# ZhengyiLuo/UHC

Hardware: NVIDIA H100
Metric: env_steps_per_s (higher is better)
Workload: dtype f32

## Files before the change

### include/uhc_b200.h

```cpp
#ifndef UHC_B200_H
#define UHC_B200_H
#ifdef __cplusplus
extern "C" {
#endif

#define UHC_NB 24
#define UHC_NQ 76
#define UHC_NV 75
#define UHC_NU 69
#define UHC_OBS_DIM 657
#define UHC_ACT_DIM 105
#define UHC_MAX_ACT_DIM 315
#define UHC_OBS_DIM_V1 784
#define UHC_EX_SIZE 576
#define UHC_BODYF 20

typedef struct UhcEngine UhcEngine;

typedef struct {
    int nvert, nnbr;
    const double *body_f;
    const double *dof_f;
    const double *hull;
    const int *hull_adr, *hull_num, *nbr, *nbradr;
// ... 38 lines not shown
int uhc_load_motions_time(const UhcEngine *e, float *out2);

int uhc_set_clip_models(UhcEngine *e, int nclips, const int *clip_model);

int uhc_set_neutral_pose(UhcEngine *e, const double *qpos76, const double *qvel75);

int uhc_set_clip_weights(UhcEngine *e, int nclips, const float *weights_host);
int uhc_get_clip_cdf(UhcEngine *e, float *out_host);

int uhc_env_reset(UhcEngine *e, int n, const int *env_ids_host, const int *clip_host, const int *start_host, const int *len_host,
                  const float *qpos_dev, const float *qvel_dev, float *obs_dev, void *stream);

int uhc_env_step(UhcEngine *e, const float *actions_dev, float *obs_dev, float *reward_dev, float *cinfo_dev, int *fail_dev,
                 int *end_dev, float *percent_dev, float *torque_dev, void *stream);

int uhc_env_step_host(UhcEngine *e, const float *actions_host, float *obs_host, float *reward_host, float *cinfo_host,
                      int *fail_host, int *end_host, float *percent_host);

int uhc_env_get_state(UhcEngine *e, int env, double *qpos76, double *qvel75, double *xpos72, double *bquat96, int *istate8);
int uhc_env_set_state(UhcEngine *e, int env, const double *qpos76, const double *qvel75);
int uhc_env_get_state_batch(UhcEngine *e, int n, const int *env_ids_host, double *out_host, int *istate_host);
int uhc_env_set_state_batch(UhcEngine *e, int n, const int *env_ids_host, const double *qpos_host, const double *qvel_host);
int uhc_engine_counters(UhcEngine *e, int *out4);
const int *uhc_episode_log_dev(const UhcEngine *e);
int uhc_num_envs(const UhcEngine *e);
int uhc_engine_obs_dim(const UhcEngine *e);
int uhc_engine_act_dim(const UhcEngine *e);
int uhc_kernel_launches(const UhcEngine *e);

#ifdef __cplusplus
}
#endif
#endif
```

### uhc_b200/build.py

```python
import os
import subprocess
import tempfile

HERE = os.path.dirname(os.path.abspath(__file__))
SO = os.path.join(HERE, "libuhc_b200.so")
SRCS = ["step_kernel.cu", "nn_kernels.cu", "mlp_wgmma.cu", "rollout.cu", "ppo_update.cu"]
NO_FMA_SRCS = ["motion_lib.cu", "eval.cu", "curriculum.cu", "track.cu", "export.cu"]
DEPS = ["sim_core.h", "env_step.h", "motion_core.h", "eval_core.h", "eval_glue.h", "group_core.h", "curriculum_core.h", "track_core.h", "track_obs.h", "track_glue.h", "smpl_export_core.h", "../../include/uhc_b200.h", "../../include/uhc_nn.h", "../../include/uhc_rollout.h", "../../include/uhc_ppo.h", "../../include/uhc_eval.h", "../../include/uhc_track.h", "../../include/uhc_export.h"]
NVCC_FLAGS = ["-gencode", "arch=compute_90a,code=sm_90a", "-O3", "-lineinfo", "-std=c++17", "--use_fast_math=false",
              "-Xcompiler", "-fPIC", "-shared", "-Xptxas", "-v", "--expt-relaxed-constexpr"]


def build(force=False, verbose=False):
    csrc = os.path.join(HERE, "csrc")
    srcs = [os.path.join(csrc, s) for s in SRCS]
    nofma = [os.path.join(csrc, s) for s in NO_FMA_SRCS]
    deps = srcs + nofma + [os.path.join(csrc, d) for d in DEPS] + [os.path.abspath(__file__)]
    if not force and os.path.exists(SO) and os.path.getmtime(SO) >= max(os.path.getmtime(d) for d in deps if os.path.exists(d)):
        return SO
    flags = [f for f in NVCC_FLAGS if f != "--use_fast_math=false"] + os.environ.get("UHC_NVCC_EXTRA", "").split()
    with tempfile.TemporaryDirectory() as tmp:
        objs = []
        for s in nofma:
            o = os.path.join(tmp, os.path.basename(s) + ".o")
            cmd = ["nvcc"] + [f for f in flags if f != "-shared"] + ["-fmad=false", "-c", "-o", o, s]
            r = subprocess.run(cmd, capture_output=True, text=True)
            if verbose or r.returncode:
                print(r.stdout[-6000:], r.stderr[-12000:])
            if r.returncode:
                raise RuntimeError("nvcc failed")
            objs.append(o)
        cmd = ["nvcc"] + flags + ["-o", SO] + srcs + objs + ["-ldl"]
        r = subprocess.run(cmd, capture_output=True, text=True)
    if verbose or r.returncode:
        print(r.stdout[-6000:], r.stderr[-12000:])
    if r.returncode:
        raise RuntimeError("nvcc failed")
    return SO


if __name__ == "__main__":
    build(force=True, verbose=True)
```

### uhc_b200/csrc/env_step.h

```cpp
#pragma once
#include "sim_core.h"
#include "curriculum_core.h"

namespace uhc {

struct CurView {
    const float *pct;
    const int *start;
    const int *meta;
    int max_freq, fit_clip;
    float prec_freq;
};

template <class Real>
struct EngineView {
    Model<Real> model;
    EnvCfg<Real> cfg;
    int num_envs;
    Real *state;
    int *istate;
    const Real *expert;
    const int *clip_adr;
    const Real *clip_shape;
    const int *clip_model;
// ... 100 lines not shown
UHC_DEV unsigned smem_u32(const void *p) { return (unsigned)__cvta_generic_to_shared(p); }
template <class Real>
UHC_DEV void state_mbar_init(Work<Real> &w) {
    if ((threadIdx.x & 31) == 0) {
        asm volatile("mbarrier.init.shared::cta.b64 [%0], 1;" :: "r"(smem_u32(&w.mbar)));
        asm volatile("fence.mbarrier_init.release.cluster;" ::: "memory");
    }
    __syncwarp();
}
template <class Real>
UHC_DEV void copy16(Real *dst, const Real *src, int n) {
    const int nv = n * (int)sizeof(Real) / 16;
    for (int i = threadIdx.x & 31; i < nv; i += 32) reinterpret_cast<uint4 *>(dst)[i] = reinterpret_cast<const uint4 *>(src)[i];
}
#endif
template <class Real>
UHC_DEV void load_state(const EngineView<Real> &ev, int env, Work<Real> &w, int parity) {
    const Real *st = ev.state + (size_t)env * ST_SIZE;
#ifndef UHC_EMU
    constexpr unsigned BYTES = ST_BLOCK * sizeof(Real);
    static_assert(BYTES % 16 == 0 && (ST_SIZE * sizeof(Real)) % 16 == 0, "bulk copies need 16-byte granularity");
    const unsigned mb = smem_u32(&w.mbar);
    if ((threadIdx.x & 31) == 0) {
        asm volatile("mbarrier.arrive.expect_tx.shared::cta.b64 _, [%0], %1;" :: "r"(mb), "r"(BYTES) : "memory");
        asm volatile("cp.async.bulk.shared::cluster.global.mbarrier::complete_tx::bytes [%0], [%1], %2, [%3];"
                     :: "r"(smem_u32(w.q)), "l"(st), "r"(BYTES), "r"(mb) : "memory");
    }
    unsigned done = 0;
    while (!done) {
        asm volatile("{ .reg .pred p; mbarrier.try_wait.parity.shared::cta.b64 p, [%1], %2; selp.u32 %0, 1, 0, p; }" : "=r"(done) : "r"(mb), "r"(parity) : "memory");
    }
    __syncwarp();
#else
    (void)parity;
    { Real *head = reinterpret_cast<Real *>(&w); for (int i = 0; i < ST_BLOCK; i++) head[i] = st[i]; }
#endif
}
template <class Real>
UHC_DEV void store_state(const EngineView<Real> &ev, int env, Work<Real> &w) {
    Real *st = ev.state + (size_t)env * ST_SIZE;
#ifndef UHC_EMU
    constexpr unsigned BYTES = ST_BLOCK * sizeof(Real);
    __syncwarp();
    copy16(st + ST_XPOS, &w.xpos[0][0], 72); copy16(st + ST_XIPOS, &w.xipos[0][0], 72); copy16(st + ST_XQUAT, &w.xquat[0][0], 96);
    if ((threadIdx.x & 31) == 0) {
        asm volatile("fence.proxy.async.shared::cta;" ::: "memory");
// ... 34 lines not shown
    }
    LANES_BEGIN
    if (lane == 0) { w.mdl = model_for_clip(ev, clip); w.cfg = ev.cfg; w.con_overflow = 0; }
    LANES_END
    const Model<Real> &mdl = w.mdl;
    TOPO_DECL(mdl);
    const int iters = substep_dynamics<Real, ObsT>(mdl, w.cfg, w, tp, (const Real *)nullptr, 0, false, (ObsT *)nullptr);
    world_quat(mdl, w.q, w);
    int *is = ev.istate + (size_t)env * SI_SIZE;
    Real *st = ev.state + (size_t)env * ST_SIZE;
    LANES_BEGIN
    for (int i = lane; i < 96; i += 32) { const Real v = (i & 3) == 0 ? Real(1) : Real(0); st[ST_BQUAT + i] = v; st[ST_PBQUAT + i] = v; }
    if (lane == 0) { is[SI_CUR_T] = 0; is[SI_CLIP] = clip; is[SI_START] = start; is[SI_LEN] = len; is[SI_NEWTON] = iters; is[SI_NCON] = w.ncon; }
    LANES_END
    if (obs) write_obs(ev, w, clip, start, len, 1, obs);
    LANES_BEGIN
    for (int i = lane; i < NV; i += 32) w.aw[i] = 0;
    LANES_END
    store_state(ev, env, w);
}

template <class Real, class ObsT, bool CUR = false>
UHC_DEV int env_step_warp(const EngineView<Real> &ev, int env, Work<Real> &w, const ObsT *action, ObsT *obs, ObsT *reward,
                          ObsT *cinfo_out, int *fail_out, int *end_out, ObsT *percent_out, ObsT *torque_out) {
    int *is = ev.istate + (size_t)env * SI_SIZE;
    Real *st = ev.state + (size_t)env * ST_SIZE;
    const int clip = is[SI_CLIP], start = is[SI_START], len = is[SI_LEN];
    int cur_t = is[SI_CUR_T];
    load_state(ev, env, w, 0);
    const bool explicit_rf = ev.cfg.rfc_mode == 1;
    LANES_BEGIN
    for (int i = lane; i < NU; i += 32) w.act[i] = (Real)action[i];
    if (lane < 6) w.act[NU + lane] = ev.cfg.rfc_mode == 0 ? (Real)action[NU + lane] : Real(0);
    if (lane < 2 * NSUB) w.act[NU + 6 + lane] = ev.cfg.meta_pd ? (Real)action[NU + ev.cfg.vf_dim + lane] : Real(0);
    LANES_END
    if (explicit_rf) restore_stale_pose(w, st + ST_XPOS, st + ST_XQUAT);
    const Real *target = expert_frame(ev, clip, start, len, cur_t + 1) + EX_QPOS + 7;
    int iters = 0, maxcon = 0;
    LANES_BEGIN
    if (lane == 0) { w.mdl = model_for_clip(ev, clip); w.cfg = ev.cfg; w.con_overflow = 0; }
    LANES_END
    const Model<Real> &mdl = w.mdl;
    TOPO_DECL(mdl);
#pragma unroll 1
    for (int it = 0; it < NSUB; ++it) {
        UHC_CTA_SYNC(true);
        iters += substep_dynamics<Real, ObsT>(mdl, w.cfg, w, tp, target, it, true, torque_out, true, action);
        if (w.ncon > maxcon) maxcon = w.ncon;
        if (it == NSUB - 1) world_quat(mdl, w.q, w);
        integrate(mdl, w);
    }
    cur_t += 1;
    Real *bq = st + ST_BQUAT, *pbq = st + ST_PBQUAT;
    LANES_BEGIN
    for (int i = lane; i < 96; i += 32) pbq[i] = bq[i];
    LANES_END
    body_quat(w, bq);
    Real bd, rew, ci[5];
    const Real *exf = expert_frame(ev, clip, start, len, cur_t);
    diff_and_reward(mdl, w.cfg, w, exf, bq, pbq, &bd, &rew, ci, action);
    int fail;
    if (ev.cfg.term_body == 0) fail = bd > ev.cfg.body_diff_thresh;
    else {
        const Real *f0 = ev.expert + (size_t)(UHC_LDG(ev.clip_adr + clip) + start) * EX_SIZE;
        const int off = ev.cfg.term_body == 1 ? EX_QPOS + 2 : EX_WBPOS + 3 * ev.cfg.head_body + 2;
        LVAR(Real, neg);
        LANES_BEGIN
        Real mx = Real(-1e30);
        for (int i = lane; i < len; i += 32) { const Real z = -(Real)UHC_LDG(f0 + (size_t)i * EX_SIZE + off); mx = z > mx ? z : mx; }
        LV(neg) = mx;
        LANES_END
        const Real lb = -WMAX(neg);
        fail = (ev.cfg.term_body == 1 ? w.q[2] : w.xpos[ev.cfg.head_body][2]) < lb - Real(0.1);
// ... 25 lines not shown
            const float pctf = (float)((Real)cur_t / (Real)(len - 1));
            ev.ep_log[2 * env] = (fail || end) ? clip : -1;
#ifndef UHC_EMU
            ev.ep_log[2 * env + 1] = __float_as_int(pctf);
#else
            union { float f; int i; } cv; cv.f = pctf; ev.ep_log[2 * env + 1] = cv.i;
#endif
            if constexpr (CUR) ev.ep_start_log[env] = start;
        }
    }
    if (cinfo_out && lane < 5) cinfo_out[lane] = (ObsT)ci[lane];
    LANES_END
    store_state(ev, env, w);
    if (ev.cfg.auto_reset && (fail || end)) {
        int nclip, nstart, nlen;
        const int episode = is[SI_EPISODE] + 1;
        if constexpr (CUR) sample_clip_cur(ev, env, episode, &nclip, &nstart, &nlen);
        else sample_clip(ev, env, episode, &nclip, &nstart, &nlen);
        env_reset_warp<Real, ObsT>(ev, env, w, nclip, nstart, nlen, (const Real *)nullptr, (const Real *)nullptr, obs);
        LANES_BEGIN
        if (lane == 0) is[SI_EPISODE] = episode;
        LANES_END
    }
    return fail || end;
}

}
```

### uhc_b200/csrc/sim_core.h

```cpp
#pragma once
#include <math.h>
#include <stdint.h>

#ifndef UHC_EMU
#include <cuda_runtime.h>
#define UHC_DEV __device__ __forceinline__
#define UHC_DEVNI __device__ __noinline__
#define LANES_BEGIN { const int lane = (int)(threadIdx.x & 31);
#define LANES_END } __syncwarp();
#define LANES_END_R }
#define LVAR(T, n) T n
#define LV(n) n
#define LVARA(T, n, K) T n[K]
#define LVA(n) n
#define LV_ARR(n, c) n[c]
#define LV_ALL(n) n
#define UHC_LDG(p) __ldg(p)
__device__ __forceinline__ float uhc_lds(const float *p) { float v; asm("ld.shared.f32 %0, [%1];" : "=f"(v) : "r"((unsigned)__cvta_generic_to_shared(p))); return v; }
__device__ __forceinline__ double uhc_lds(const double *p) { double v; asm("ld.shared.f64 %0, [%1];" : "=d"(v) : "r"((unsigned)__cvta_generic_to_shared(p))); return v; }
__device__ __forceinline__ int uhc_lds(const int *p) { int v; asm("ld.shared.s32 %0, [%1];" : "=r"(v) : "r"((unsigned)__cvta_generic_to_shared(p))); return v; }
#define UHC_LDT(p) uhc_lds(p)
#else
#define UHC_DEV static inline
#define UHC_DEVNI static
// ... 1088 lines not shown
    const Real dt = m.dt;
    LANES_BEGIN
    for (int i = lane; i < NV; i += 32) { const Real vn = w.v[i] + dt * w.a[i]; w.v[i] = vn; w.aw[i] = w.a[i]; if (i >= 6) w.q[i + 1] += dt * vn; }
    LANES_END
    LANES_BEGIN
    if (lane < 3) w.q[lane] += dt * w.v[lane];
    if (lane == 3) {
        const Real wx = w.v[3], wy = w.v[4], wz = w.v[5], n = sqrt(wx * wx + wy * wy + wz * wz), ang = n * dt;
        Real dq[4] = {1, 0, 0, 0}, qn[4], qo[4] = {w.q[3], w.q[4], w.q[5], w.q[6]};
        if (ang > Real(1e-30)) { Real sn, cs; sincos_(Real(0.5) * ang, &sn, &cs); const Real s = sn / n; dq[0] = cs; dq[1] = wx * s; dq[2] = wy * s; dq[3] = wz * s; }
        qmul(qo, dq, qn);
        const Real nn = rsqrt_(qn[0] * qn[0] + qn[1] * qn[1] + qn[2] * qn[2] + qn[3] * qn[3]);
        for (int i = 0; i < 4; i++) w.q[3 + i] = qn[i] * nn;
    }
    LANES_END
}

enum { PH_PD = 0, PH_SMOOTH = 1, PH_NEWTON = 2 };
#if !defined(UHC_EMU) && !defined(UHC_NO_CTA_SYNC)
#define UHC_CTA_SYNC(on) do { if (on) asm volatile("bar.sync %0, %1;" :: "r"(w.sync_id), "r"(w.sync_threads) : "memory"); } while (0)
#else
#define UHC_CTA_SYNC(on) do { (void)(on); } while (0)
#endif
template <class Real, class OutT, class TPT>
UHC_DEVNI int substep_dynamics(const Model<Real> &m, const EnvCfg<Real> &cfg, Work<Real> &w, const TPT &tp, const Real *target, int it,
                             bool with_pd, OutT *torque_out, bool cta_sync = false, const OutT *act_global = nullptr) {
    int phase = with_pd ? PH_PD : PH_SMOOTH, iters = 0;
    bool done = false;
    Real scale = 0, gn2 = 0;
    for (;;) {
        Real *rhs = w.p;
        Real arm_scale = 0;
        if (phase == PH_PD) {
            pd_setup(m, cfg, w, target, it);
            Real sp, sd; pd_gains(cfg, w, it, &sp, &sd);
            arm_scale = sd * m.dt;
        } else if (phase == PH_SMOOTH) {
            Real fapp[6] = {0, 0, 0, 0, 0, 0};
            const bool explicit_rf = with_pd && cfg.rfc_mode == 1 && act_global != nullptr;
            if (explicit_rf) rfc_explicit(m, cfg, w, tp, act_global, w.as_);
            else if (with_pd && cfg.rfc_mode == 0) rfc_implicit(cfg, w, fapp);
            kin_rne_forward(m, w, tp);
            project_force(m, w, w.Fb, w.C, Real(1), (const Real *)nullptr);
            collide(m, w, tp);
            LANES_BEGIN
            for (int i = lane; i < NV; i += 32) {
                Real f = -w.C[i];
                if (explicit_rf) f += w.as_[i];
                else if (i < 6) { const Real fa = i == 0 ? fapp[0] : i == 1 ? fapp[1] : i == 2 ? fapp[2] : i == 3 ? fapp[3] : i == 4 ? fapp[4] : fapp[5]; f += fa; }
                if (i >= 6 && with_pd) f += w.tau[i - 6];
                w.fs[i] = f; w.as_[i] = f;
            }
            LANES_END
            rhs = w.as_;
            limit_setup(m, w);
        } else {
            if (done || iters >= cfg.newton_max_iter || !(gn2 > cfg.newton_tol * cfg.newton_tol * scale * scale)) break;
            ++iters;
        }
        if (!(phase == PH_SMOOTH && (w.ncon > 0 || w.nlim > 0))) aba_solve(m, w, arm_scale, phase == PH_NEWTON, rhs);
        if (phase == PH_PD) { pd_finish(m, cfg, w, it, torque_out); phase = PH_SMOOTH; UHC_CTA_SYNC(cta_sync); }
        else if (phase == PH_SMOOTH) {
            UHC_CTA_SYNC(cta_sync);
            if (w.ncon == 0 && w.nlim == 0) {
                LANES_BEGIN
                for (int i = lane; i < NV; i += 32) w.a[i] = w.as_[i];
                LANES_END
                done = true;
            } else {
                constraint_setup(m, w);
                scale = newton_init(m, w, tp, &gn2);
            }
            phase = PH_NEWTON;
        } else if (newton_advance(m, w, tp, &gn2)) done = true;
    }
    return iters;
}

template <class Real>
UHC_DEVNI void body_quat(const Work<Real> &w, Real *out) {
    LANES_BEGIN
    const int b = lane;
    if (b == 0) for (int i = 0; i < 4; i++) out[i] = w.q[3 + i];
    else if (b < NB) euler_zyx_quat(w.q[7 + 3 * (b - 1)], w.q[8 + 3 * (b - 1)], w.q[9 + 3 * (b - 1)], out + 4 * b);
    LANES_END
}
template <class Real>
UHC_DEVNI void world_quat(const Model<Real> &m, const Real *qfk, Work<Real> &w) {
    LANES_BEGIN
    const int b = lane;
    if (b < NB) {
        int chain[MAXLEVEL + 1], n = 0;
        for (int a = b; a > 0; a = UHC_LDG(m.parent + a)) chain[n++] = a;
        Real q[4] = {qfk[3], qfk[4], qfk[5], qfk[6]};
        const Real nn = rsqrt_(q[0] * q[0] + q[1] * q[1] + q[2] * q[2] + q[3] * q[3]);
// ... 209 lines not shown
```

### uhc_b200/csrc/step_kernel.cu

```cuda
#include <cuda_runtime.h>
#include <stdio.h>
#include <stdlib.h>
#include <string.h>
#include <string>
#include <vector>
#include "../../include/uhc_b200.h"
#include "../../include/uhc_rollout.h"
#include "env_step.h"
#include "motion_core.h"
#include "eval_glue.h"
#include "curriculum_core.h"
#include "track_obs.h"
#include "track_glue.h"

using namespace uhc;

static thread_local std::string g_err;
#define CK(x) do { cudaError_t e_ = (x); if (e_ != cudaSuccess) { g_err = std::string(#x) + ": " + cudaGetErrorString(e_); return -1; } } while (0)

template <class Real, int EPB>
__device__ __forceinline__ void stage_tables(EngineView<Real> &ev, unsigned char *smem) {
    Real *s_dof = reinterpret_cast<Real *>(smem + EPB * sizeof(Work<Real>));
    Real *s_lim = s_dof + NV * 4;
    int *s_lvl = reinterpret_cast<int *>(s_lim + NV * 4);
    for (int i = threadIdx.x; i < NV * 4; i += blockDim.x) { s_dof[i] = ev.model.dof_f[i]; s_lim[i] = ev.model.dof_lim[i]; }
    for (int i = threadIdx.x; i < (MAXLEVEL + 1) * LVL_G; i += blockDim.x) s_lvl[i] = ev.model.lvl_pack[i];
    LaneTopo *s_topo = reinterpret_cast<LaneTopo *>(s_lvl + (MAXLEVEL + 1) * LVL_G);
    if (threadIdx.x < 32) s_topo[threadIdx.x] = lane_topo(ev.model, (int)threadIdx.x);
    __syncthreads();
    ev.model.dof_f = s_dof; ev.model.dof_lim = s_lim; ev.model.lvl_pack = s_lvl; ev.model.topo_s = s_topo;
}

constexpr int SYNC_GROUP = 8;
#ifdef UHC_MAXNREG
#define UHC_STEP_BOUNDS(EPB, Real) __maxnreg__(UHC_MAXNREG)
#else
#define UHC_STEP_BOUNDS(EPB, Real) __launch_bounds__(32 * EPB, 1)
#endif
template <class Real, int EPB, bool CUR = false>
__global__ void UHC_STEP_BOUNDS(EPB, Real)
k_env_step(EngineView<Real> ev, const float *__restrict__ act, float *__restrict__ obs, float *__restrict__ rew, float *__restrict__ cinfo,
           int *__restrict__ fail, int *__restrict__ end, float *__restrict__ pct, float *__restrict__ torque, const int *__restrict__ order) {
    extern __shared__ __align__(16) unsigned char smem[];
    constexpr int NGRP = (EPB + SYNC_GROUP - 1) / SYNC_GROUP;
    __shared__ int s_nvalid[NGRP];
    const int warp = threadIdx.x >> 5, slot = blockIdx.x * EPB + warp, grp = warp / SYNC_GROUP;
    if (threadIdx.x < NGRP) s_nvalid[threadIdx.x] = 0;
    stage_tables<Real, EPB>(ev, smem);
    const int env = slot < ev.num_envs ? (order ? order[slot] : slot) : -1;
    const bool valid = env >= 0 && env_record_valid(ev, env);
    if (valid && (threadIdx.x & 31) == 0) atomicAdd(&s_nvalid[grp], 1);
    __syncthreads();
    if (!valid) {
        if (env >= 0) env_step_invalid<Real, float>(ev, obs ? obs + (size_t)env * ev.cfg.obs_dim : nullptr, rew ? rew + env : nullptr, cinfo ? cinfo + (size_t)env * 5 : nullptr,
                                                    fail ? fail + env : nullptr, end ? end + env : nullptr, pct ? pct + env : nullptr);
        return;
    }
    Work<Real> &w = reinterpret_cast<Work<Real> *>(smem)[warp];
    if ((threadIdx.x & 31) == 0) { w.sync_threads = 32 * s_nvalid[grp]; w.sync_id = 1 + grp; }
    state_mbar_init(w);
    env_step_warp<Real, float, CUR>(ev, env, w, act + (size_t)env * ev.cfg.act_dim, obs ? obs + (size_t)env * ev.cfg.obs_dim : nullptr, rew ? rew + env : nullptr,
                               cinfo ? cinfo + (size_t)env * 5 : nullptr, fail ? fail + env : nullptr, end ? end + env : nullptr,
                               pct ? pct + env : nullptr, torque ? torque + (size_t)env * NSUB * NU : nullptr);
}

__global__ void __launch_bounds__(1024) k_order_envs(const int *__restrict__ istate, int E, int *__restrict__ order) {
    __shared__ int hist[64], base[64];
    if (threadIdx.x < 64) hist[threadIdx.x] = 0;
    __syncthreads();
    for (int i = threadIdx.x; i < E; i += blockDim.x) { int k = istate[(size_t)i * SI_SIZE + SI_NEWTON]; k = k < 0 ? 0 : (k > 63 ? 63 : k); atomicAdd(&hist[k], 1); }
    __syncthreads();
    if (threadIdx.x == 0) { int run = 0; for (int k = 0; k < 64; k++) { base[k] = run; run += hist[k]; } }
    __syncthreads();
    for (int i = threadIdx.x; i < E; i += blockDim.x) { int k = istate[(size_t)i * SI_SIZE + SI_NEWTON]; k = k < 0 ? 0 : (k > 63 ? 63 : k); order[atomicAdd(&base[k], 1)] = i; }
}

template <class Real, int EPB>
__global__ void __launch_bounds__(32 * EPB)
k_env_reset(EngineView<Real> ev, int n, const int *__restrict__ ids, const int *__restrict__ clip, const int *__restrict__ start,
            const int *__restrict__ len, const float *__restrict__ qpos, const float *__restrict__ qvel, float *__restrict__ obs) {
    extern __shared__ __align__(16) unsigned char smem[];
    const int warp = threadIdx.x >> 5, i = blockIdx.x * EPB + warp;
    stage_tables<Real, EPB>(ev, smem);
    if (i >= n) return;
    Work<Real> &w = reinterpret_cast<Work<Real> *>(smem)[warp];
    const int env = ids[i];
// ... 59 lines not shown
template <class Real>
__global__ void k_gather_state(const Real *__restrict__ state, const int *__restrict__ istate, const int *__restrict__ ids, int n, double *__restrict__ out, int *__restrict__ iout) {
    const int i = blockIdx.x; if (i >= n) return;
    const int env = ids[i];
    const Real *st = state + (size_t)env * ST_SIZE;
    double *o = out + (size_t)i * 319;
    for (int k = threadIdx.x; k < NQ; k += blockDim.x) o[k] = (double)st[ST_Q + k];
    for (int k = threadIdx.x; k < NV; k += blockDim.x) o[76 + k] = (double)st[ST_V + k];
    for (int k = threadIdx.x; k < 72; k += blockDim.x) o[151 + k] = (double)st[ST_XPOS + k];
    for (int k = threadIdx.x; k < 96; k += blockDim.x) o[223 + k] = (double)st[ST_BQUAT + k];
    if (threadIdx.x < SI_SIZE) iout[(size_t)i * SI_SIZE + threadIdx.x] = istate[(size_t)env * SI_SIZE + threadIdx.x];
}
template <class Real>
__global__ void k_save_restore_bquat(Real *__restrict__ state, int *__restrict__ istate, const int *__restrict__ ids, int n, Real *__restrict__ keep, int *__restrict__ keep_t, int restore) {
    const int i = blockIdx.x; if (i >= n) return;
    const int env = ids[i];
    Real *st = state + (size_t)env * ST_SIZE + ST_BQUAT;
    for (int k = threadIdx.x; k < 192; k += blockDim.x) { if (restore) st[k] = keep[(size_t)i * 192 + k]; else keep[(size_t)i * 192 + k] = st[k]; }
    if (threadIdx.x == 0) { if (restore) istate[(size_t)env * SI_SIZE + SI_CUR_T] = keep_t[i]; else keep_t[i] = istate[(size_t)env * SI_SIZE + SI_CUR_T]; }
}

struct UhcEngine {
    int E, device, precision, launches;
    std::vector<void *> allocs;
    EngineView<float> evf; EngineView<double> evd;
    int *d_clip_model = nullptr; int nshape = 1;
    void *d_expert = nullptr, *d_shape = nullptr; int *d_clip_adr = nullptr; float *d_clip_cdf = nullptr; int num_clips = 0;
    float *d_act = nullptr, *d_obs = nullptr, *d_rew = nullptr, *d_cinfo = nullptr, *d_pct = nullptr; int *d_fail = nullptr, *d_end = nullptr;
    int *d_ids = nullptr; int ids_cap = 0;
    int *h_ids = nullptr;
    cudaEvent_t ids_done = nullptr;
    float *d_qv = nullptr; int qv_cap = 0; void *d_keep = nullptr; int *d_keep_t = nullptr;
    double *d_gather = nullptr; int *d_gather_i = nullptr; int gather_cap = 0;
    std::vector<float> clip_w;
    int *d_order = nullptr;
    std::vector<int> clip_len_h;
    std::vector<int> clip_adr_h;
    unsigned long long view_gen = 0;
    unsigned long long table_gen = 0;
    motion::MotionModel mo_model;
    float mo_ms[2] = {0.f, 0.f};
    cur::Dev cur = {};
    float prec_freq = 0.f; int fit_clip = -1;
    unsigned long long cur_gen = 0;
    size_t cur_cnt_cap = 0, cur_rank_cap = 0;
    int *d_reseed = nullptr;
// ... 45 lines not shown
#undef CPI
    M.dt = (Real)m->dt; M.margin = (Real)m->margin; M.mu = (Real)m->mu; M.solref0 = (Real)m->solref[0]; M.solref1 = (Real)m->solref[1];
    M.simp0 = (Real)m->solimp[0]; M.simp1 = (Real)m->solimp[1]; M.simp2 = (Real)m->solimp[2]; M.simp3 = (Real)m->solimp[3]; M.simp4 = (Real)m->solimp[4];
    M.gravz = (Real)m->gravz;
    fill_cfg(ev.cfg, cfg);
    ev.num_envs = e->E;
    Real *st; CK(cudaMalloc((void **)&st, (size_t)e->E * ST_SIZE * sizeof(Real))); e->allocs.push_back(st);
    CK(cudaMemset(st, 0, (size_t)e->E * ST_SIZE * sizeof(Real)));
    int *is; CK(cudaMalloc((void **)&is, (size_t)e->E * SI_SIZE * sizeof(int))); e->allocs.push_back(is);
    CK(cudaMemset(is, 0, (size_t)e->E * SI_SIZE * sizeof(int)));
    int *cn; CK(cudaMalloc((void **)&cn, 4 * sizeof(int))); e->allocs.push_back(cn); CK(cudaMemset(cn, 0, 4 * sizeof(int)));
    ev.counters = cn; ev.neutral = nullptr;
    int *el; CK(cudaMalloc((void **)&el, (size_t)e->E * 3 * sizeof(int))); e->allocs.push_back(el); CK(cudaMemset(el, 0xFF, (size_t)e->E * 3 * sizeof(int)));
    ev.ep_log = el; ev.ep_start_log = el + (size_t)2 * e->E;
    ev.cur.pct = nullptr; ev.cur.start = nullptr; ev.cur.meta = nullptr; ev.cur.max_freq = 0; ev.cur.fit_clip = -1; ev.cur.prec_freq = 0.f;
    ev.state = st; ev.istate = is; ev.expert = nullptr; ev.clip_adr = nullptr; ev.clip_shape = nullptr; ev.clip_model = nullptr; ev.clip_cdf = nullptr;
    return 0;
}

constexpr int EPB_F = 16, EPB_D = 2;
template <class Real, int EPB> constexpr size_t step_smem() { return EPB * sizeof(Work<Real>) + 2 * NV * 4 * sizeof(Real) + (MAXLEVEL + 1) * LVL_G * sizeof(int) + 32 * sizeof(LaneTopo); }
static_assert(step_smem<float, EPB_F>() + 1024 + 64 <= 228 * 1024, "k_env_step<float>: the 16 work sets of a block no longer fit one SM");

extern "C" {

const char *uhc_last_error(void) { return g_err.c_str(); }

int uhc_engine_create(const UhcModelHost *model, const UhcEnvCfg *cfg, int num_envs, int device, int precision, UhcEngine **out) {
    if (!model || !cfg || !out || num_envs <= 0 || (precision != 32 && precision != 64)) { g_err = "uhc_engine_create: bad argument"; return -2; }
    CK(cudaSetDevice(device));
    UhcEngine *e = new UhcEngine();
    e->E = num_envs; e->device = device; e->precision = precision; e->launches = 0; e->nshape = model->nshape > 0 ? model->nshape : 1;
    int rc = precision == 32 ? build_view<float>(e, e->evf, model, cfg) : build_view<double>(e, e->evd, model, cfg);
    if (rc) { delete e; return rc; }
    {
        std::vector<double> body((size_t)e->nshape * NB * motion::BODY6);
        motion::motion_body_table(model->body_f, BODYF, e->nshape, body.data());
        double *d_body;
        if (dev_copy(e, &d_body, body.data(), body.size())) { delete e; return -1; }
        motion::motion_model_init(e->mo_model, model->parent, model->ee, d_body);
    }
    {
        const char *se = getenv("UHC_SORT_ENVS");
        if (se && se[0] == '1' && num_envs > 2 * EPB_F) { CK(cudaMalloc((void **)&e->d_order, (size_t)num_envs * sizeof(int))); e->allocs.push_back(e->d_order); }
    }
    if (precision == 32) {
        CK(cudaFuncSetAttribute(k_env_step<float, EPB_F>, cudaFuncAttributeMaxDynamicSharedMemorySize, (int)step_smem<float, EPB_F>()));
        CK(cudaFuncSetAttribute(k_env_step<float, EPB_F, true>, cudaFuncAttributeMaxDynamicSharedMemorySize, (int)step_smem<float, EPB_F>()));
        CK(cudaFuncSetAttribute(k_env_reset<float, EPB_F>, cudaFuncAttributeMaxDynamicSharedMemorySize, (int)step_smem<float, EPB_F>()));
        CK(cudaFuncSetAttribute(k_eval_reseat<float, EPB_F>, cudaFuncAttributeMaxDynamicSharedMemorySize, (int)step_smem<float, EPB_F>()));
        int resident = 0;
        CK(cudaOccupancyMaxActiveBlocksPerMultiprocessor(&resident, k_env_step<float, EPB_F>, 32 * EPB_F, step_smem<float, EPB_F>()));
        if (resident < 1) { g_err = "uhc_engine_create: k_env_step<float> with " + std::to_string(EPB_F) + " envs per block does not fit one SM"; delete e; return -3; }
    } else {
        CK(cudaFuncSetAttribute(k_env_step<double, EPB_D>, cudaFuncAttributeMaxDynamicSharedMemorySize, (int)step_smem<double, EPB_D>()));
        CK(cudaFuncSetAttribute(k_env_step<double, EPB_D, true>, cudaFuncAttributeMaxDynamicSharedMemorySize, (int)step_smem<double, EPB_D>()));
        CK(cudaFuncSetAttribute(k_env_reset<double, EPB_D>, cudaFuncAttributeMaxDynamicSharedMemorySize, (int)step_smem<double, EPB_D>()));
        CK(cudaFuncSetAttribute(k_eval_reseat<double, EPB_D>, cudaFuncAttributeMaxDynamicSharedMemorySize, (int)step_smem<double, EPB_D>()));
    }
    const size_t E = num_envs;
    CK(cudaMalloc((void **)&e->d_act, E * MAX_ACT_DIM * 4)); CK(cudaMalloc((void **)&e->d_obs, E * (size_t)(precision == 32 ? e->evf.cfg.obs_dim : e->evd.cfg.obs_dim) * 4)); CK(cudaMalloc((void **)&e->d_rew, E * 4));
    CK(cudaMalloc((void **)&e->d_cinfo, E * 5 * 4)); CK(cudaMalloc((void **)&e->d_pct, E * 4)); CK(cudaMalloc((void **)&e->d_fail, E * 4)); CK(cudaMalloc((void **)&e->d_end, E * 4));
    for (void *p : {(void *)e->d_act, (void *)e->d_obs, (void *)e->d_rew, (void *)e->d_cinfo, (void *)e->d_pct, (void *)e->d_fail, (void *)e->d_end}) e->allocs.push_back(p);
    *out = e;
    return 0;
}

void uhc_engine_destroy(UhcEngine *e) {
    if (!e) return;
    cudaSetDevice(e->device);
    for (void *p : e->allocs) cudaFree(p);
    if (e->d_expert) cudaFree(e->d_expert);
    if (e->d_shape) cudaFree(e->d_shape);
    if (e->d_clip_adr) cudaFree(e->d_clip_adr);
    if (e->d_clip_cdf) cudaFree(e->d_clip_cdf);
    if (e->d_clip_model) cudaFree(e->d_clip_model);
// ... 250 lines not shown
    }
    memcpy(e->h_ids, env_ids_host, n * sizeof(int)); memcpy(e->h_ids + n, clip_host, n * sizeof(int));
    memcpy(e->h_ids + 2 * n, start_host, n * sizeof(int)); memcpy(e->h_ids + 3 * n, len_host, n * sizeof(int));
    CK(cudaMemcpyAsync(e->d_ids, e->h_ids, (size_t)4 * n * sizeof(int), cudaMemcpyHostToDevice, st));
    if (e->precision == 32)
        k_env_reset<float, EPB_F><<<(n + EPB_F - 1) / EPB_F, 32 * EPB_F, step_smem<float, EPB_F>(), st>>>(e->evf, n, e->d_ids, e->d_ids + n, e->d_ids + 2 * n, e->d_ids + 3 * n, qpos_dev, qvel_dev, obs_dev);
    else
        k_env_reset<double, EPB_D><<<(n + EPB_D - 1) / EPB_D, 32 * EPB_D, step_smem<double, EPB_D>(), st>>>(e->evd, n, e->d_ids, e->d_ids + n, e->d_ids + 2 * n, e->d_ids + 3 * n, qpos_dev, qvel_dev, obs_dev);
    CK(cudaGetLastError());
    CK(cudaEventRecord(e->ids_done, st));
    e->launches++;
    return 0;
}

int uhc_env_step(UhcEngine *e, const float *actions_dev, float *obs_dev, float *reward_dev, float *cinfo_dev, int *fail_dev, int *end_dev,
                 float *percent_dev, float *torque_dev, void *stream) {
    if (!e || !actions_dev) { g_err = "uhc_env_step: bad argument"; return -2; }
    if (!e->d_expert) { g_err = "uhc_env_step: no clips loaded"; return -3; }
    CK(cudaSetDevice(e->device));
    cudaStream_t st = (cudaStream_t)stream;
    if (e->d_order) { k_order_envs<<<1, 1024, 0, st>>>(e->precision == 32 ? e->evf.istate : e->evd.istate, e->E, e->d_order); e->launches++; }
    const bool cur = e->cur.M > 0;
    if (e->precision == 32)
        (cur ? k_env_step<float, EPB_F, true> : k_env_step<float, EPB_F>)<<<(e->E + EPB_F - 1) / EPB_F, 32 * EPB_F, step_smem<float, EPB_F>(), st>>>(e->evf, actions_dev, obs_dev, reward_dev, cinfo_dev, fail_dev, end_dev, percent_dev, torque_dev, e->d_order);
    else
        (cur ? k_env_step<double, EPB_D, true> : k_env_step<double, EPB_D>)<<<(e->E + EPB_D - 1) / EPB_D, 32 * EPB_D, step_smem<double, EPB_D>(), st>>>(e->evd, actions_dev, obs_dev, reward_dev, cinfo_dev, fail_dev, end_dev, percent_dev, torque_dev, e->d_order);
    CK(cudaGetLastError());
    e->launches++;
    return 0;
}

int uhc_env_step_host(UhcEngine *e, const float *actions_host, float *obs_host, float *reward_host, float *cinfo_host, int *fail_host,
                      int *end_host, float *percent_host) {
    if (!e || !actions_host) { g_err = "uhc_env_step_host: bad argument"; return -2; }
    CK(cudaSetDevice(e->device));
    const size_t E = e->E;
    CK(cudaMemcpyAsync(e->d_act, actions_host, E * (size_t)uhc_engine_act_dim(e) * 4, cudaMemcpyHostToDevice, 0));
    int rc = uhc_env_step(e, e->d_act, e->d_obs, e->d_rew, e->d_cinfo, e->d_fail, e->d_end, e->d_pct, nullptr, nullptr);
    if (rc) return rc;
    if (obs_host) CK(cudaMemcpyAsync(obs_host, e->d_obs, E * (size_t)uhc_engine_obs_dim(e) * 4, cudaMemcpyDeviceToHost, 0));
    if (reward_host) CK(cudaMemcpyAsync(reward_host, e->d_rew, E * 4, cudaMemcpyDeviceToHost, 0));
    if (cinfo_host) CK(cudaMemcpyAsync(cinfo_host, e->d_cinfo, E * 5 * 4, cudaMemcpyDeviceToHost, 0));
    if (fail_host) CK(cudaMemcpyAsync(fail_host, e->d_fail, E * 4, cudaMemcpyDeviceToHost, 0));
    if (end_host) CK(cudaMemcpyAsync(end_host, e->d_end, E * 4, cudaMemcpyDeviceToHost, 0));
    if (percent_host) CK(cudaMemcpyAsync(percent_host, e->d_pct, E * 4, cudaMemcpyDeviceToHost, 0));
    CK(cudaStreamSynchronize(0));
    return 0;
// ... 58 lines not shown
    int *d_idl = e->d_keep_t + n;
    CK(cudaMemcpy(d_idl, env_ids_host, n * sizeof(int), cudaMemcpyHostToDevice));
    if (e->precision == 32) k_save_restore_bquat<float><<<n, 64>>>(e->evf.state, e->evf.istate, d_idl, n, (float *)e->d_keep, e->d_keep_t, 0);
    else k_save_restore_bquat<double><<<n, 64>>>(e->evd.state, e->evd.istate, d_idl, n, (double *)e->d_keep, e->d_keep_t, 0);
    rc = uhc_env_reset(e, n, env_ids_host, clip.data(), start.data(), len.data(), e->d_qv, e->d_qv + (size_t)n * NQ, nullptr, nullptr);
    if (rc) return rc;
    if (e->precision == 32) k_save_restore_bquat<float><<<n, 64>>>(e->evf.state, e->evf.istate, d_idl, n, (float *)e->d_keep, e->d_keep_t, 1);
    else k_save_restore_bquat<double><<<n, 64>>>(e->evd.state, e->evd.istate, d_idl, n, (double *)e->d_keep, e->d_keep_t, 1);
    CK(cudaGetLastError());
    CK(cudaDeviceSynchronize());
    return 0;
}

int uhc_env_set_state(UhcEngine *e, int env, const double *qpos76, const double *qvel75) {
    return uhc_env_set_state_batch(e, 1, &env, qpos76, qvel75);
}

int uhc_engine_counters(UhcEngine *e, int *out4) {
    if (!e || !out4) { g_err = "uhc_engine_counters: bad argument"; return -2; }
    CK(cudaSetDevice(e->device));
    CK(cudaDeviceSynchronize());
    CK(cudaMemcpy(out4, e->precision == 32 ? e->evf.counters : e->evd.counters, 4 * sizeof(int), cudaMemcpyDeviceToHost));
    return 0;
}

const int *uhc_episode_log_dev(const UhcEngine *e) { return e ? (e->precision == 32 ? e->evf.ep_log : e->evd.ep_log) : nullptr; }
int uhc_num_envs(const UhcEngine *e) { return e ? e->E : -1; }
int uhc_engine_obs_dim(const UhcEngine *e) { return e ? (e->precision == 32 ? e->evf.cfg.obs_dim : e->evd.cfg.obs_dim) : -1; }
int uhc_engine_act_dim(const UhcEngine *e) { return e ? (e->precision == 32 ? e->evf.cfg.act_dim : e->evd.cfg.act_dim) : -1; }
int uhc_kernel_launches(const UhcEngine *e) { return e ? e->launches : -1; }

static void cur_view(UhcEngine *e) {
    CurView v;
    v.pct = e->cur.pct; v.start = e->cur.start; v.meta = e->cur.meta; v.max_freq = e->cur.M;
    v.fit_clip = e->cur.M ? e->fit_clip : -1; v.prec_freq = e->cur.M ? e->prec_freq : 0.f;
    e->evf.cur = v; e->evd.cur = v;
    e->view_gen++; e->cur_gen++;
}
static void cur_free(UhcEngine *e) {
    cudaDeviceSynchronize();
    for (void *p : {(void *)e->cur.pct, (void *)e->cur.start, (void *)e->cur.meta, (void *)e->cur.p, (void *)e->cur.cnt, (void *)e->cur.rank, (void *)e->cur.ncl}) if (p) cudaFree(p);
    if (e->d_push) cudaFree(e->d_push);
    e->d_push = nullptr; e->push_cap = 0;
    e->cur = cur::Dev{}; e->cur_cnt_cap = e->cur_rank_cap = 0; e->fit_clip = -1; e->prec_freq = 0.f;
    int *sl = e->precision == 32 ? e->evf.ep_start_log : e->evd.ep_start_log;
    cudaMemset(sl, 0xFF, (size_t)e->E * sizeof(int));
// ... 240 lines not shown
```

Baseline: 1.272 million.

## Cap step grid at resident CTAs and loop each block over multiple env rounds

The float step kernel now launches at most one wave of resident CTAs, with a floor of a quarter of the env blocks. Each block loops over up to four rounds of env slots, reusing staged tables and alternating mbarrier parity, with a separate named barrier per round group. This is meant to cut repeated per-block table staging and tail-wave imbalance. It also adds optional clock64 phase instrumentation compiled in only with UHC_STEP_CLOCKS, plus an async proxy fence before the bulk state load.

```diff
diff --git a/include/uhc_b200.h b/include/uhc_b200.h
--- a/include/uhc_b200.h
+++ b/include/uhc_b200.h
@@ -84,6 +84,7 @@
 int uhc_env_get_state_batch(UhcEngine *e, int n, const int *env_ids_host, double *out_host, int *istate_host);
 int uhc_env_set_state_batch(UhcEngine *e, int n, const int *env_ids_host, const double *qpos_host, const double *qvel_host);
 int uhc_engine_counters(UhcEngine *e, int *out4);
+int uhc_step_clocks(UhcEngine *e, int nslots, unsigned long long *out_host, int *rec_len);
 const int *uhc_episode_log_dev(const UhcEngine *e);
 int uhc_num_envs(const UhcEngine *e);
 int uhc_engine_obs_dim(const UhcEngine *e);
diff --git a/uhc_b200/build.py b/uhc_b200/build.py
--- a/uhc_b200/build.py
+++ b/uhc_b200/build.py
@@ -11,14 +11,15 @@
               "-Xcompiler", "-fPIC", "-shared", "-Xptxas", "-v", "--expt-relaxed-constexpr"]
 
 
-def build(force=False, verbose=False):
+def build(force=False, verbose=False, so=None, extra_flags=()):
+    so = so or SO
     csrc = os.path.join(HERE, "csrc")
     srcs = [os.path.join(csrc, s) for s in SRCS]
     nofma = [os.path.join(csrc, s) for s in NO_FMA_SRCS]
     deps = srcs + nofma + [os.path.join(csrc, d) for d in DEPS] + [os.path.abspath(__file__)]
-    if not force and os.path.exists(SO) and os.path.getmtime(SO) >= max(os.path.getmtime(d) for d in deps if os.path.exists(d)):
-        return SO
-    flags = [f for f in NVCC_FLAGS if f != "--use_fast_math=false"] + os.environ.get("UHC_NVCC_EXTRA", "").split()
+    if not force and os.path.exists(so) and os.path.getmtime(so) >= max(os.path.getmtime(d) for d in deps if os.path.exists(d)):
+        return so
+    flags = [f for f in NVCC_FLAGS if f != "--use_fast_math=false"] + os.environ.get("UHC_NVCC_EXTRA", "").split() + list(extra_flags)
     with tempfile.TemporaryDirectory() as tmp:
         objs = []
         for s in nofma:
@@ -30,13 +31,13 @@
             if r.returncode:
                 raise RuntimeError("nvcc failed")
             objs.append(o)
-        cmd = ["nvcc"] + flags + ["-o", SO] + srcs + objs + ["-ldl"]
+        cmd = ["nvcc"] + flags + ["-o", so] + srcs + objs + ["-ldl"]
         r = subprocess.run(cmd, capture_output=True, text=True)
     if verbose or r.returncode:
         print(r.stdout[-6000:], r.stderr[-12000:])
     if r.returncode:
         raise RuntimeError("nvcc failed")
-    return SO
+    return so
 
 
 if __name__ == "__main__":
diff --git a/uhc_b200/csrc/env_step.h b/uhc_b200/csrc/env_step.h
--- a/uhc_b200/csrc/env_step.h
+++ b/uhc_b200/csrc/env_step.h
@@ -146,6 +146,7 @@
     static_assert(BYTES % 16 == 0 && (ST_SIZE * sizeof(Real)) % 16 == 0, "bulk copies need 16-byte granularity");
     const unsigned mb = smem_u32(&w.mbar);
     if ((threadIdx.x & 31) == 0) {
+        asm volatile("fence.proxy.async.shared::cta;" ::: "memory");
         asm volatile("mbarrier.arrive.expect_tx.shared::cta.b64 _, [%0], %1;" :: "r"(mb), "r"(BYTES) : "memory");
         asm volatile("cp.async.bulk.shared::cluster.global.mbarrier::complete_tx::bytes [%0], [%1], %2, [%3];"
                      :: "r"(smem_u32(w.q)), "l"(st), "r"(BYTES), "r"(mb) : "memory");
@@ -226,12 +227,12 @@
 
 template <class Real, class ObsT, bool CUR = false>
 UHC_DEV int env_step_warp(const EngineView<Real> &ev, int env, Work<Real> &w, const ObsT *action, ObsT *obs, ObsT *reward,
-                          ObsT *cinfo_out, int *fail_out, int *end_out, ObsT *percent_out, ObsT *torque_out) {
+                          ObsT *cinfo_out, int *fail_out, int *end_out, ObsT *percent_out, ObsT *torque_out, int load_parity = 0) {
     int *is = ev.istate + (size_t)env * SI_SIZE;
     Real *st = ev.state + (size_t)env * ST_SIZE;
     const int clip = is[SI_CLIP], start = is[SI_START], len = is[SI_LEN];
     int cur_t = is[SI_CUR_T];
-    load_state(ev, env, w, 0);
+    load_state(ev, env, w, load_parity);
     const bool explicit_rf = ev.cfg.rfc_mode == 1;
     LANES_BEGIN
     for (int i = lane; i < NU; i += 32) w.act[i] = (Real)action[i];
@@ -246,13 +247,16 @@
     LANES_END
     const Model<Real> &mdl = w.mdl;
     TOPO_DECL(mdl);
+    UHC_CLK(true, CLK_PROLOGUE);
 #pragma unroll 1
     for (int it = 0; it < NSUB; ++it) {
         UHC_CTA_SYNC(true);
+        UHC_CLK(true, CLK_BAR_START);
         iters += substep_dynamics<Real, ObsT>(mdl, w.cfg, w, tp, target, it, true, torque_out, true, action);
         if (w.ncon > maxcon) maxcon = w.ncon;
         if (it == NSUB - 1) world_quat(mdl, w.q, w);
         integrate(mdl, w);
+        UHC_CLK(true, CLK_INTEGRATE);
     }
     cur_t += 1;
     Real *bq = st + ST_BQUAT, *pbq = st + ST_PBQUAT;
@@ -324,6 +328,7 @@
         if (lane == 0) is[SI_EPISODE] = episode;
         LANES_END
     }
+    UHC_CLK(true, CLK_EPILOGUE);
     return fail || end;
 }
 
diff --git a/uhc_b200/csrc/sim_core.h b/uhc_b200/csrc/sim_core.h
--- a/uhc_b200/csrc/sim_core.h
+++ b/uhc_b200/csrc/sim_core.h
@@ -1134,6 +1134,21 @@
 #else
 #define UHC_CTA_SYNC(on) do { (void)(on); } while (0)
 #endif
+enum { CLK_PROLOGUE = 0, CLK_BAR_START, CLK_PD, CLK_BAR_PD, CLK_SMOOTH, CLK_BAR_SMOOTH, CLK_NEWTON_SETUP, CLK_NEWTON, CLK_INTEGRATE, CLK_EPILOGUE,
+       CLK_NPH, CLK_T0 = CLK_NPH, CLK_LAST, CLK_GROUP, CLK_ITERS, CLK_REC = CLK_ITERS + NSUB };
+#if defined(UHC_STEP_CLOCKS) && !defined(UHC_EMU)
+constexpr int CLK_SLOTS = 8192;
+static __device__ unsigned long long g_step_clk[CLK_SLOTS * CLK_REC];
+__device__ __forceinline__ unsigned long long *clk_rec() {
+    const unsigned slot = blockIdx.x * (blockDim.x >> 5) + (threadIdx.x >> 5);
+    return (threadIdx.x & 31) == 0 && slot < CLK_SLOTS ? g_step_clk + (size_t)slot * CLK_REC : nullptr;
+}
+#define UHC_CLK(on, ph) do { unsigned long long *r_ = clk_rec(); if ((on) && r_) { const unsigned long long t_ = clock64(); r_[ph] += t_ - r_[CLK_LAST]; r_[CLK_LAST] = t_; } } while (0)
+#define UHC_CLK_SET(on, k, v) do { unsigned long long *r_ = clk_rec(); if ((on) && r_) r_[k] = (unsigned long long)(v); } while (0)
+#else
+#define UHC_CLK(on, ph) do { } while (0)
+#define UHC_CLK_SET(on, k, v) do { } while (0)
+#endif
 template <class Real, class OutT, class TPT>
 UHC_DEVNI int substep_dynamics(const Model<Real> &m, const EnvCfg<Real> &cfg, Work<Real> &w, const TPT &tp, const Real *target, int it,
                              bool with_pd, OutT *torque_out, bool cta_sync = false, const OutT *act_global = nullptr) {
@@ -1167,13 +1182,18 @@
             rhs = w.as_;
             limit_setup(m, w);
         } else {
-            if (done || iters >= cfg.newton_max_iter || !(gn2 > cfg.newton_tol * cfg.newton_tol * scale * scale)) break;
+            if (done || iters >= cfg.newton_max_iter || !(gn2 > cfg.newton_tol * cfg.newton_tol * scale * scale)) {
+                UHC_CLK(cta_sync, CLK_NEWTON); UHC_CLK_SET(cta_sync, CLK_ITERS + it, iters);
+                break;
+            }
             ++iters;
         }
         if (!(phase == PH_SMOOTH && (w.ncon > 0 || w.nlim > 0))) aba_solve(m, w, arm_scale, phase == PH_NEWTON, rhs);
-        if (phase == PH_PD) { pd_finish(m, cfg, w, it, torque_out); phase = PH_SMOOTH; UHC_CTA_SYNC(cta_sync); }
-        else if (phase == PH_SMOOTH) {
-            UHC_CTA_SYNC(cta_sync);
+        if (phase == PH_PD) {
+            pd_finish(m, cfg, w, it, torque_out); phase = PH_SMOOTH;
+            UHC_CLK(cta_sync, CLK_PD); UHC_CTA_SYNC(cta_sync); UHC_CLK(cta_sync, CLK_BAR_PD);
+        } else if (phase == PH_SMOOTH) {
+            UHC_CLK(cta_sync, CLK_SMOOTH); UHC_CTA_SYNC(cta_sync); UHC_CLK(cta_sync, CLK_BAR_SMOOTH);
             if (w.ncon == 0 && w.nlim == 0) {
                 LANES_BEGIN
                 for (int i = lane; i < NV; i += 32) w.a[i] = w.as_[i];
@@ -1183,6 +1203,7 @@
                 constraint_setup(m, w);
                 scale = newton_init(m, w, tp, &gn2);
             }
+            UHC_CLK(cta_sync, CLK_NEWTON_SETUP);
             phase = PH_NEWTON;
         } else if (newton_advance(m, w, tp, &gn2)) done = true;
     }
diff --git a/uhc_b200/csrc/step_kernel.cu b/uhc_b200/csrc/step_kernel.cu
--- a/uhc_b200/csrc/step_kernel.cu
+++ b/uhc_b200/csrc/step_kernel.cu
@@ -37,31 +37,44 @@
 #else
 #define UHC_STEP_BOUNDS(EPB, Real) __launch_bounds__(32 * EPB, 1)
 #endif
+constexpr int STEP_ROUNDS = 4;
 template <class Real, int EPB, bool CUR = false>
 __global__ void UHC_STEP_BOUNDS(EPB, Real)
 k_env_step(EngineView<Real> ev, const float *__restrict__ act, float *__restrict__ obs, float *__restrict__ rew, float *__restrict__ cinfo,
            int *__restrict__ fail, int *__restrict__ end, float *__restrict__ pct, float *__restrict__ torque, const int *__restrict__ order) {
     extern __shared__ __align__(16) unsigned char smem[];
     constexpr int NGRP = (EPB + SYNC_GROUP - 1) / SYNC_GROUP;
-    __shared__ int s_nvalid[NGRP];
-    const int warp = threadIdx.x >> 5, slot = blockIdx.x * EPB + warp, grp = warp / SYNC_GROUP;
-    if (threadIdx.x < NGRP) s_nvalid[threadIdx.x] = 0;
+    static_assert(1 + STEP_ROUNDS * NGRP <= 16, "named barriers 1..15");
+    __shared__ int s_nvalid[STEP_ROUNDS * NGRP];
+    const int warp = threadIdx.x >> 5, grp = warp / SYNC_GROUP;
+    const int nblk = (ev.num_envs + EPB - 1) / EPB, rounds = (nblk + (int)gridDim.x - 1) / (int)gridDim.x;
+    UHC_CLK_SET(true, CLK_T0, clock64()); UHC_CLK_SET(true, CLK_LAST, clock64());
+    if (threadIdx.x < STEP_ROUNDS * NGRP) s_nvalid[threadIdx.x] = 0;
     stage_tables<Real, EPB>(ev, smem);
-    const int env = slot < ev.num_envs ? (order ? order[slot] : slot) : -1;
-    const bool valid = env >= 0 && env_record_valid(ev, env);
-    if (valid && (threadIdx.x & 31) == 0) atomicAdd(&s_nvalid[grp], 1);
+    auto env_of = [&](int r) { const int slot = (blockIdx.x + r * gridDim.x) * EPB + warp; return slot < ev.num_envs ? (order ? order[slot] : slot) : -1; };
+    for (int r = 0; r < rounds; ++r) {
+        const int env = env_of(r);
+        if (env >= 0 && env_record_valid(ev, env) && (threadIdx.x & 31) == 0) atomicAdd(&s_nvalid[r * NGRP + grp], 1);
+    }
     __syncthreads();
-    if (!valid) {
-        if (env >= 0) env_step_invalid<Real, float>(ev, obs ? obs + (size_t)env * ev.cfg.obs_dim : nullptr, rew ? rew + env : nullptr, cinfo ? cinfo + (size_t)env * 5 : nullptr,
-                                                    fail ? fail + env : nullptr, end ? end + env : nullptr, pct ? pct + env : nullptr);
-        return;
-    }
     Work<Real> &w = reinterpret_cast<Work<Real> *>(smem)[warp];
-    if ((threadIdx.x & 31) == 0) { w.sync_threads = 32 * s_nvalid[grp]; w.sync_id = 1 + grp; }
     state_mbar_init(w);
-    env_step_warp<Real, float, CUR>(ev, env, w, act + (size_t)env * ev.cfg.act_dim, obs ? obs + (size_t)env * ev.cfg.obs_dim : nullptr, rew ? rew + env : nullptr,
-                               cinfo ? cinfo + (size_t)env * 5 : nullptr, fail ? fail + env : nullptr, end ? end + env : nullptr,
-                               pct ? pct + env : nullptr, torque ? torque + (size_t)env * NSUB * NU : nullptr);
+    int loads = 0;
+    for (int r = 0; r < rounds; ++r) {
+        const int env = env_of(r);
+        if (env < 0) continue;
+        if (!env_record_valid(ev, env)) {
+            env_step_invalid<Real, float>(ev, obs ? obs + (size_t)env * ev.cfg.obs_dim : nullptr, rew ? rew + env : nullptr, cinfo ? cinfo + (size_t)env * 5 : nullptr,
+                                          fail ? fail + env : nullptr, end ? end + env : nullptr, pct ? pct + env : nullptr);
+            continue;
+        }
+        if ((threadIdx.x & 31) == 0) { w.sync_threads = 32 * s_nvalid[r * NGRP + grp]; w.sync_id = 1 + r * NGRP + grp; }
+        UHC_CLK_SET(true, CLK_GROUP, grp);
+        env_step_warp<Real, float, CUR>(ev, env, w, act + (size_t)env * ev.cfg.act_dim, obs ? obs + (size_t)env * ev.cfg.obs_dim : nullptr, rew ? rew + env : nullptr,
+                                   cinfo ? cinfo + (size_t)env * 5 : nullptr, fail ? fail + env : nullptr, end ? end + env : nullptr,
+                                   pct ? pct + env : nullptr, torque ? torque + (size_t)env * NSUB * NU : nullptr, loads & 1);
+        ++loads;
+    }
 }
 
 __global__ void __launch_bounds__(1024) k_order_envs(const int *__restrict__ istate, int E, int *__restrict__ order) {
@@ -167,6 +180,7 @@
 
 struct UhcEngine {
     int E, device, precision, launches;
+    int step_ctas = 0;
     std::vector<void *> allocs;
     EngineView<float> evf; EngineView<double> evd;
     int *d_clip_model = nullptr; int nshape = 1;
@@ -258,6 +272,12 @@
 template <class Real, int EPB> constexpr size_t step_smem() { return EPB * sizeof(Work<Real>) + 2 * NV * 4 * sizeof(Real) + (MAXLEVEL + 1) * LVL_G * sizeof(int) + 32 * sizeof(LaneTopo); }
 static_assert(step_smem<float, EPB_F>() + 1024 + 64 <= 228 * 1024, "k_env_step<float>: the 16 work sets of a block no longer fit one SM");
 
+static int step_grid(int E, int epb, int ctas) {
+    const int nblk = (E + epb - 1) / epb;
+    const int g = nblk < ctas ? nblk : ctas, lo = (nblk + STEP_ROUNDS - 1) / STEP_ROUNDS;
+    return g > lo ? g : lo;
+}
+
 extern "C" {
 
 const char *uhc_last_error(void) { return g_err.c_str(); }
@@ -288,6 +308,9 @@
         int resident = 0;
         CK(cudaOccupancyMaxActiveBlocksPerMultiprocessor(&resident, k_env_step<float, EPB_F>, 32 * EPB_F, step_smem<float, EPB_F>()));
         if (resident < 1) { g_err = "uhc_engine_create: k_env_step<float> with " + std::to_string(EPB_F) + " envs per block does not fit one SM"; delete e; return -3; }
+        int nsm = 0;
+        CK(cudaDeviceGetAttribute(&nsm, cudaDevAttrMultiProcessorCount, device));
+        e->step_ctas = resident * nsm;
     } else {
         CK(cudaFuncSetAttribute(k_env_step<double, EPB_D>, cudaFuncAttributeMaxDynamicSharedMemorySize, (int)step_smem<double, EPB_D>()));
         CK(cudaFuncSetAttribute(k_env_step<double, EPB_D, true>, cudaFuncAttributeMaxDynamicSharedMemorySize, (int)step_smem<double, EPB_D>()));
@@ -584,7 +607,7 @@
     if (e->d_order) { k_order_envs<<<1, 1024, 0, st>>>(e->precision == 32 ? e->evf.istate : e->evd.istate, e->E, e->d_order); e->launches++; }
     const bool cur = e->cur.M > 0;
     if (e->precision == 32)
-        (cur ? k_env_step<float, EPB_F, true> : k_env_step<float, EPB_F>)<<<(e->E + EPB_F - 1) / EPB_F, 32 * EPB_F, step_smem<float, EPB_F>(), st>>>(e->evf, actions_dev, obs_dev, reward_dev, cinfo_dev, fail_dev, end_dev, percent_dev, torque_dev, e->d_order);
+        (cur ? k_env_step<float, EPB_F, true> : k_env_step<float, EPB_F>)<<<step_grid(e->E, EPB_F, e->step_ctas), 32 * EPB_F, step_smem<float, EPB_F>(), st>>>(e->evf, actions_dev, obs_dev, reward_dev, cinfo_dev, fail_dev, end_dev, percent_dev, torque_dev, e->d_order);
     else
         (cur ? k_env_step<double, EPB_D, true> : k_env_step<double, EPB_D>)<<<(e->E + EPB_D - 1) / EPB_D, 32 * EPB_D, step_smem<double, EPB_D>(), st>>>(e->evd, actions_dev, obs_dev, reward_dev, cinfo_dev, fail_dev, end_dev, percent_dev, torque_dev, e->d_order);
     CK(cudaGetLastError());
@@ -689,6 +712,23 @@
     CK(cudaDeviceSynchronize());
     CK(cudaMemcpy(out4, e->precision == 32 ? e->evf.counters : e->evd.counters, 4 * sizeof(int), cudaMemcpyDeviceToHost));
     return 0;
+}
+
+int uhc_step_clocks(UhcEngine *e, int nslots, unsigned long long *out_host, int *rec_len) {
+    if (rec_len) *rec_len = CLK_REC;
+#ifdef UHC_STEP_CLOCKS
+    if (!e || nslots < 0 || nslots > CLK_SLOTS || (nslots && !out_host)) { g_err = "uhc_step_clocks: bad argument"; return -2; }
+    CK(cudaSetDevice(e->device));
+    const size_t bytes = (size_t)nslots * CLK_REC * sizeof(unsigned long long);
+    CK(cudaMemcpyFromSymbol(out_host, g_step_clk, bytes));
+    std::vector<unsigned long long> zero((size_t)CLK_SLOTS * CLK_REC, 0ull);
+    CK(cudaMemcpyToSymbol(g_step_clk, zero.data(), zero.size() * sizeof(unsigned long long)));
+    return 0;
+#else
+    (void)e; (void)nslots; (void)out_host;
+    g_err = "uhc_step_clocks: this library was built without -DUHC_STEP_CLOCKS";
+    return -4;
+#endif
 }
 
 const int *uhc_episode_log_dev(const UhcEngine *e) { return e ? (e->precision == 32 ? e->evf.ep_log : e->evd.ep_log) : nullptr; }
```

Result: no change. 1.278 million, median of 6 (+0.5%).
